# youshyee/CoSA

Measured on AMD Instinct MI355X. Metric: training images/sec at 448x448 ViT-B, higher is better.
Workload: dtype bf16; 1 GPU; VOC12 21-class, ViT-B/16 bf16, batch 16/GPU x 448x448, teacher 3 scales x 2 flips + student fwd/bwd + cam2mask x2 + 5 losses + AdamW + EMA; global_batch=16, parallelism=dp1, defer_groups=1, grid_policy=full grid

## Files before the change

### cosa_amd/csrc/gemm_kernels.hip

```cpp
#include "kernels.hpp"
#include "op16.hpp"
#include "c8.hpp"
#include "c4.hpp"
#include <cstdlib>

namespace cosa {
namespace {

typedef float f32x4 __attribute__((ext_vector_type(4)));

constexpr int BM = 128, BN = 128, BK = 64;
constexpr int TILE_BYTES = 128 * BK * 2;
constexpr int STAGE_BYTES = 2 * TILE_BYTES;
constexpr int CT_LD = 272;

enum { EPI_BIAS = 0, EPI_GELU = 1, EPI_RESIDUAL = 2 };

__device__ __forceinline__ float gelu_erf(float x)
{
    const float z = __builtin_fabsf(x) * 0.70710678118654752f;
    const float t = __builtin_amdgcn_rcpf(__builtin_fmaf(0.3275911f, z, 1.0f));
    float p = __builtin_fmaf(1.061405429f, t, -1.453152027f);
    p = __builtin_fmaf(p, t, 1.421413741f);
    p = __builtin_fmaf(p, t, -0.284496736f);
    p = __builtin_fmaf(p, t, 0.254829592f);
    p = p * t;
    const float e = __builtin_amdgcn_exp2f(-z * z * 1.4426950408889634f);
    const float erf_abs = __builtin_fmaf(-p, e, 1.0f);
    const float erfx = __builtin_copysignf(erf_abs, x);
    return 0.5f * x * (1.0f + erfx);
}

#define COSA_SPLIT_OPAQUE(a, b) asm volatile("" : "+v"(a), "+v"(b))

typedef __attribute__((address_space(3))) void lds_void;
typedef const __attribute__((address_space(1))) void gbl_void;

__device__ __forceinline__ void stage_tile(const op16 *__restrict__ src, int row0, int nrows, int ld, int k0,
                                           unsigned char *lds_tile, int wave, int lane)
{
#pragma unroll
    for (int i = 0; i < 4; i++) {
        const int q = wave * 4 + i;
        const int row = 8 * q + (lane >> 3);
        const int s = (lane & 7) ^ (row & 7);
        int grow = row0 + row;
        grow = grow < nrows ? grow : nrows - 1;
        const op16 *g = src + (size_t)grow * ld + k0 + s * 8;
        __builtin_amdgcn_global_load_lds((gbl_void *)g, (lds_void *)(lds_tile + q * 1024), 16, 0, 0);
    }
}

struct SplitGeom { int Kp; };
__device__ __forceinline__ int split_tile_x(int kt, int Kp) { return kt <= 2 * Kp ? kt : kt - 2 * Kp - 1; }
__device__ __forceinline__ int split_tile_w(int kt, int Kp) { return kt < Kp ? kt : (kt < 2 * Kp ? kt - Kp : (kt == 2 * Kp ? kt : kt - Kp - 1)); }

__device__ __forceinline__ bool c8_is_f8(int kt, int Kp) { return kt > Kp; }
__device__ __forceinline__ int c8_tile_x(int kt, int Kp) { return kt < Kp ? kt : (kt == Kp ? 2 * Kp : kt - 1); }
__device__ __forceinline__ int c8_tile_w(int kt, int Kp)
{
    const int Kh = Kp >> 1;
    return kt < Kp ? kt : (kt == Kp ? 2 * Kp : (kt <= Kp + Kh ? kt + Kh - 1 : kt - Kh - 1));
}
typedef int c8_i32x8 __attribute__((ext_vector_type(8)));
typedef int c8_i32x4 __attribute__((ext_vector_type(4)));
__device__ __forceinline__ c8_i32x8 c8_cat(op16x8 lo, op16x8 hi)
{
    return __builtin_shufflevector(__builtin_bit_cast(c8_i32x4, lo), __builtin_bit_cast(c8_i32x4, hi), 0, 1, 2, 3, 4, 5, 6, 7);
}
constexpr int kC8ScaleW = 0x7f7f7f7f;
constexpr int kC8ScaleX = 0x74747474;
#define COSA_MFMA_C8(a8, b8, c) __builtin_amdgcn_mfma_scale_f32_16x16x128_f8f6f4(a8, b8, c, 1, 1, 0, kC8ScaleW, 0, kC8ScaleX)

template <int OA, int OB>
__device__ __forceinline__ f32x4 mfma_c4(c8_i32x8 a4, c8_i32x8 b4, f32x4 c, int sa, int sb)
{
    return __builtin_amdgcn_mfma_scale_f32_16x16x128_f8f6f4(a4, b4, c, 4, 4, OA, sa, OB, sb);
}
__device__ __forceinline__ c8_i32x8 c4_op(op16x8 v)
{
    const c8_i32x4 t = __builtin_bit_cast(c8_i32x4, v);
    return (c8_i32x8){t[0], t[1], t[2], t[3], 0, 0, 0, 0};
}
__device__ __forceinline__ float c4_max4(float v)
{
    const unsigned u = __builtin_bit_cast(unsigned, v);
    const auto a = __builtin_amdgcn_permlane16_swap(u, u, false, false);
    const unsigned m = a[0] > a[1] ? a[0] : a[1];
// ... 24 lines not shown
        if (m0 >= M) return;
    } else {
        const int nwg = tiles_m * tiles_n;
        int wg = blockIdx.x;
        {
            const int q = nwg >> 3, r = nwg & 7, xcd = wg & 7, idx = wg >> 3;
            wg = (xcd < r ? xcd * (q + 1) : r * (q + 1) + (xcd - r) * q) + idx;
        }
        const int tm = wg / tiles_n, tn = wg - tm * tiles_n;
        m0 = tm * BM;
        n0 = tn * BN;
    }
    const int wr = wave >> 1, wc = wave & 1;

    f32x4 acc[4][4];
    const bool tail = tail_o0 >= 0;
#pragma unroll
    for (int i = 0; i < 4; i++)
#pragma unroll
        for (int j = 0; j < 4; j++) {
            acc[i][j] = (f32x4){0.f, 0.f, 0.f, 0.f};
            if (tail) {
                const int nl = (wave >> 1) * 64 + 16 * i + 4 * (lane >> 4), ml = (wave & 1) * 64 + 16 * j + (lane & 15);
                if (EPI == EPI_RESIDUAL) {
                    if (m0 + ml < M) acc[i][j] = *reinterpret_cast<const f32x4 *>(R + (size_t)(m0 + ml) * N + n0 + nl);
                } else {
#pragma unroll
                    for (int r = 0; r < 4; r++) acc[i][j][r] = (float)bias[n0 + nl + r];
                }
            }
        }

    const int Kp = K / BK;
    const int nk = SPLIT == 1 ? 3 * Kp + 1 : (SPLIT == 3 ? 2 * Kp + 1 : Kp);
    auto tile_x = [&](int kt) { return SPLIT == 1 ? split_tile_x(kt, Kp) : (SPLIT == 3 ? c8_tile_x(kt, Kp) : kt); };
    auto tile_w = [&](int kt) { return SPLIT == 1 ? split_tile_w(kt, Kp) : (SPLIT == 3 ? c8_tile_w(kt, Kp) : kt); };
    stage_tile(W, n0, N, ld, 0, smem, wave, lane);
    stage_tile(X, m0, M, ld, 0, smem + TILE_BYTES, wave, lane);
    asm volatile("s_waitcnt vmcnt(0)" ::: "memory");
    __syncthreads();

    const int frow = lane & 15, fq = lane >> 4;
    for (int kt = 0; kt < nk; kt++) {
        unsigned char *cur = smem + (kt & 1) * STAGE_BYTES;
        unsigned char *nxt = smem + ((kt + 1) & 1) * STAGE_BYTES;
        if (kt + 1 < nk) {
            stage_tile(W, n0, N, ld, tile_w(kt + 1) * BK, nxt, wave, lane);
            stage_tile(X, m0, M, ld, tile_x(kt + 1) * BK, nxt + TILE_BYTES, wave, lane);
        }
        const unsigned char *At = cur + (wr * 64) * 128;
        const unsigned char *Bt = cur + TILE_BYTES + (wc * 64) * 128;
        if (SPLIT == 3 && kt > Kp) {
            op16x8 a2[4][2], b2[4][2];
#pragma unroll
            for (int i = 0; i < 4; i++) {
                const int row = i * 16 + frow;
#pragma unroll
                for (int ks = 0; ks < 2; ks++) {
                    const int slot = ((fq + 4 * ks) ^ (row & 7)) << 4;
                    a2[i][ks] = *reinterpret_cast<const op16x8 *>(At + row * 128 + slot);
                    b2[i][ks] = *reinterpret_cast<const op16x8 *>(Bt + row * 128 + slot);
                }
            }
#pragma unroll
            for (int i = 0; i < 4; i++) {
                const c8_i32x8 a8 = c8_cat(a2[i][0], a2[i][1]);
#pragma unroll
                for (int j = 0; j < 4; j++) acc[i][j] = COSA_MFMA_C8(a8, c8_cat(b2[j][0], b2[j][1]), acc[i][j]);
            }
        } else
#pragma unroll
        for (int ks = 0; ks < 2; ks++) {
            op16x8 a[4], b[4];
#pragma unroll
            for (int i = 0; i < 4; i++) {
// ... 94 lines not shown
        V5_FENCE();                           \
        __builtin_amdgcn_s_barrier();         \
        V5_FENCE();                           \
    } while (0)

typedef unsigned u32x2 __attribute__((ext_vector_type(2)));
typedef unsigned u32x4 __attribute__((ext_vector_type(4)));

template <int EPI, int SPLIT = 0, int FR = 4>
__global__ __launch_bounds__(512, 1) void gemm_bf16_v6_kernel(const op16 *__restrict__ X, const op16 *__restrict__ W,
                                                             const op16 *__restrict__ bias, const float *__restrict__ R,
                                                             void *__restrict__ Yv, int M, int N, int K, int tiles_m, int tiles_n,
                                                             unsigned long long *__restrict__ stamps, int ld, int ldy, void *__restrict__ Y2v, int ntiles_run,
                                                             const unsigned char *__restrict__ xsc, const unsigned char *__restrict__ wsc, unsigned char *__restrict__ ysc)
{
    if (stamps && threadIdx.x == 0) atomicMin(&stamps[2 * (blockIdx.x & 63)], __builtin_amdgcn_s_memrealtime());
    constexpr bool RES = EPI == EPI_RESIDUAL;
    constexpr int ES = RES ? 4 : 2;
    constexpr int FL = 0x00020000;
    static_assert(FR == 4 || (FR == 3 && SPLIT == 0), "FR: 16-feature fragments per wave and W half (tile width 64 FR)");
    constexpr bool C8 = SPLIT == 3;
    constexpr bool C8OUT = C8 && EPI == EPI_GELU;
    constexpr bool C4 = SPLIT == 4;
    constexpr bool C4OUT = C4 && EPI == EPI_GELU;
    constexpr bool CX = C8 || C4;
    static_assert(!C4 || FR == 4, "fp16c4: 256-wide jobs only (the scale tensors are laid out for them)");
    constexpr int TN = 64 * FR, HN = 32 * FR, WN = 16 * FR;
    extern __shared__ __attribute__((aligned(16))) unsigned char smem[];
    const int tid = threadIdx.x, wave = tid >> 6, lane = tid & 63;
    const int wr = wave >> 2, wc = wave & 3;
    const int frow = lane & 15, fq = lane >> 4;
    const int Kp = K / BK;
    const int Kq = Kp >> 1;
    const int nk = SPLIT == 1 ? 3 * Kp + 1 : (C8 ? 2 * Kp + 1 : (C4 ? Kp + 1 + Kq : Kp));
    const int ntiles = tiles_m * tiles_n, G = gridDim.x;
    const int cq = ntiles >> 3, cr = ntiles & 7;
    unsigned char *Yb = static_cast<unsigned char *>(Yv);

    auto tile_of = [&](int o, int &m0_, int &n0_) {
        const int xcd = o & 7, idx = o >> 3;
        const int t = (xcd < cr ? xcd * (cq + 1) : cr * (cq + 1) + (xcd - cr) * cq) + idx;
        const int tm = t / tiles_n;
        m0_ = tm * 256;
        n0_ = (t - tm * tiles_n) * TN;
    };
    auto descX = [&](int m0_) {
        int rows = M - m0_;
        rows = rows > 256 ? 256 : rows;
        return __builtin_amdgcn_make_buffer_rsrc((void *)(X + (size_t)m0_ * ld), 0, rows * ld * 2, FL);
    };
    auto descW = [&](int n0_) { return __builtin_amdgcn_make_buffer_rsrc((void *)(W + (size_t)n0_ * ld), 0, TN * ld * 2, FL); };
    auto descY2 = [&](int m0_, int n0_) {
        int rows = M - m0_;
        rows = rows > 256 ? 256 : rows;
        return __builtin_amdgcn_make_buffer_rsrc((void *)(static_cast<unsigned char *>(Y2v) + ((size_t)m0_ * ldy + n0_) * 2), 0, (rows * ldy - n0_) * 2, FL);
    };
    auto descY = [&](int m0_, int n0_) {
        int rows = M - m0_;
        rows = rows > 256 ? 256 : rows;
        return __builtin_amdgcn_make_buffer_rsrc((void *)(Yb + ((size_t)m0_ * ldy + n0_) * ES), 0, (rows * ldy - n0_) * ES, FL);
    };
    auto descR = [&](int m0_, int n0_) {
        int rows = M - m0_;
        rows = rows > 256 ? 256 : rows;
        const unsigned long long p = (unsigned long long)(R + (size_t)m0_ * N + n0_);
        return (u32x4){(unsigned)p, (unsigned)(p >> 32) & 0xffffu, (unsigned)((rows * N - n0_) * 4), (unsigned)FL};
    };
// ... 3 lines not shown
    __amdgpu_buffer_rsrc_t sXr = dead, sWr = dead, sYr = dead;
    if (C4) {
        sXr = __builtin_amdgcn_make_buffer_rsrc((void *)xsc, 0, tiles_m * Kq * 2048, FL);
        sWr = __builtin_amdgcn_make_buffer_rsrc((void *)wsc, 0, tiles_n * Kq * 2048, FL);
        if (C4OUT) sYr = __builtin_amdgcn_make_buffer_rsrc((void *)ysc, 0, tiles_m * (N >> 7) * 2048, FL);
    }
    const unsigned sc_rd_x = (unsigned)(((wc * 16 + frow) * 4 + fq) * 8), sc_rd_w = (unsigned)(4096 + ((wr * 16 + frow) * 4 + fq) * 16);
    const unsigned sc_wr_y = (unsigned)((((wc * 16 + frow) * 4 + (fq & 1) + 2 * (fq >> 1)) * 8) + wr);
    u32x2 sxv = {0, 0};
    u32x4 swv = {0, 0, 0, 0};
#define V6_SCDMA(c)                                                                                                    \
    do {                                                                                                               \
        const int c_ = (c);                                                                                            \
        const __amdgpu_buffer_rsrc_t rs_ = wave_u < 4 ? sXr : sWr;                                                     \
        const int so_ = wave_u < 4 ? (((m0 >> 8) * Kq + 2 * c_) * 2048 + wave_u * 1024) : (((n0 >> 8) * Kq + 2 * c_) * 2048 + (wave_u - 4) * 1024); \
        __builtin_amdgcn_raw_ptr_buffer_load_lds(rs_, (lds_void *)(smem + kLdsBytesV5 + (c_ & 1) * 8192 + wave_u * 1024), 16, lane * 16, so_, 0, 0); \
    } while (0)
#define V6_LDSC(q)                                                                                                     \
    do {                                                                                                               \
        const unsigned char *sb_ = smem + kLdsBytesV5 + (((q) >> 1) & 1) * 8192 + ((q) & 1) * 2048;                    \
        sxv = *reinterpret_cast<const u32x2 *>(sb_ + sc_rd_x);                                                         \
        swv = *reinterpret_cast<const u32x4 *>(sb_ + sc_rd_w);            \
    } while (0)

    unsigned vo[2][2], voW[2][2];
    {
        const int sw = ((lane & 7) ^ (lane >> 3)) * 8;
#pragma unroll
        for (int h = 0; h < 2; h++)
#pragma unroll
            for (int i = 0; i < 2; i++) {
                const int rl = 8 * (2 * wave + i) + (lane >> 3);
                vo[h][i] = (unsigned)(((h * 128 + rl) * ld + sw) * 2);
                voW[h][i] = FR == 4 ? vo[h][i] : (rl < HN ? (unsigned)(((h * HN + rl) * ld + sw) * 2) : 0x7ffff000u);
            }
    }
    const unsigned voY0 = RES ? (unsigned)(((wc * 32 + frow) * ldy + wr * WN + 4 * fq) * 4)
                              : (unsigned)(((wc * 32 + frow) * ldy + wr * WN + (fq & 1) * 16 + 4 * (fq & 2)) * 2);
    const unsigned voY3 = (unsigned)((32 + 4 * fq - (fq & 1) * 16 - 4 * (fq & 2)) * 2);
    const unsigned fo16m = (unsigned)((wr * WN + 16 * (fq & 1) + 32 * (fq >> 1)) - 2 * (wr * WN + (fq & 1) * 16 + 4 * (fq & 2)));

    constexpr bool STG = FR == 4 && EPI != EPI_GELU;
    constexpr int STGW = C4 ? 2048 : 4096;
    const unsigned stg0 = (unsigned)(kLdsBytesV5 + (C4 ? kC4ScaleLds : 0) + wave * STGW);
    const unsigned stg_w = stg0 + frow * 128 + ((((RES ? fq : (fq & 1) * 2 + (fq >> 1))) ^ (frow & 7)) << 4);
    const unsigned stg_r = stg0 + (lane >> 3) * 128 + (((lane & 7) ^ ((lane >> 3) & 7)) << 4);
    const unsigned voS = (unsigned)(((wc * 32 + (lane >> 3)) * ldy + wr * WN) * ES + (lane & 7) * 16);
#define V6_STG_WR(u4, e, plane) *reinterpret_cast<u32x4 *>(smem + ((stg_w ^ ((e) * 64)) + (plane) * 2048)) = (u4)
#define V6_STG_RD(it, plane) (*reinterpret_cast<const u32x4 *>(smem + (stg_r + (it) * 1024 + (plane) * 2048)))
    const int ldy_es = __builtin_amdgcn_readfirstlane(ldy * ES);
#define V6_VOY(g4)                                                                                                   \
    ({                                                                                                               \
        unsigned r_ = voY0;                                                                                          \
        if ((g4) != 0)                                                                                               \
            asm volatile("v_add_u32 %0, %1, %2" : "=v"(r_) : "s"((((g4) >> 1) * 128 + ((g4) & 1) * 16) * ldy_es), "v"(voY0));  \
        r_;                                                                                                          \
    })
#define V6_STG_OFF(qb, jj, it)                                                                                       \
    ({                                                                                                               \
        unsigned r_ = voS;                                                                                           \
        if ((qb) * 128 + (jj) * 16 + (it) * 8 != 0)                                                                  \
            asm volatile("v_add_u32 %0, %1, %2" : "=v"(r_) : "s"(((qb) * 128 + (jj) * 16 + (it) * 8) * ldy_es), "v"(voS));  \
        r_;                                                                                                          \
    })

    int o = blockIdx.x;
    int m0, n0, m1 = 0, n1 = 0, pn0 = 0, pm0 = 0;
    tile_of(o, m0, n0);
    bool has_next = o + G < ntiles_run;
    if (has_next) tile_of(o + G, m1, n1);
    __amdgpu_buffer_rsrc_t cX = descX(m0), cW = descW(n0), cY = descY(m0, n0), pY = cY;
    __amdgpu_buffer_rsrc_t cY2 = SPLIT == 2 ? descY2(m0, n0) : cY, pY2 = cY2;
    __amdgpu_buffer_rsrc_t nX = has_next ? descX(m1) : dead, nW = has_next ? descW(n1) : dead;
    u32x4 cR = {0, 0, 0, 0}, nR = {0, 0, 0, 0};
    if (RES) {
        cR = descR(m0, n0);
        if (has_next) nR = descR(m1, n1);
    }
    bool have_prev = false;

    u32x2 bb[2][4];
    const unsigned bias_lane = (unsigned)((wr * WN + 4 * fq) * 2);
#define V6_LOAD_BIAS(nbase)                                                                               \
    if (!CX) _Pragma("unroll") for (int a_ = 0; a_ < 2; a_++) _Pragma("unroll") for (int i_ = 0; i_ < FR; i_++) {  \
        const op16 *p_ = bias + (nbase) + a_ * HN + i_ * 16;                                              \
        asm volatile("global_load_dwordx2 %0, %1, %2" : "=v"(bb[a_][i_]) : "v"(bias_lane), "s"(p_) : "memory"); \
    }

#define V6_STAGE(which, kt, bsel)                                                                                      \
    do {                                                                                                               \
        const int kt_ = (kt);                                                                                          \
        const bool own_ = kt_ < nk;                                                                                    \
        const __amdgpu_buffer_rsrc_t rs_ = ((which) & 1) ? (own_ ? cW : nW) : (own_ ? cX : nX);                        \
        const int t_ = own_ ? kt_ : kt_ - nk;                                                                          \
        const int so_ = (SPLIT == 1 ? (((which) & 1) ? split_tile_w(t_, Kp) : split_tile_x(t_, Kp))                       \
                         : (C8 ? (((which) & 1) ? c8_tile_w(t_, Kp) : c8_tile_x(t_, Kp)) : (C4 ? c8_tile_x(t_, Kp) : t_))) * 128;   \
        unsigned char *dst_ = smem + (bsel) * V5_BUF + (which) * V5_HALF + (2 * wave) * 1024;                          \
        __builtin_amdgcn_raw_ptr_buffer_load_lds(rs_, (lds_void *)dst_, 16, ((which) & 1) ? voW[(which) >> 1][0] : vo[(which) >> 1][0], so_, 0, 0);           \
        __builtin_amdgcn_raw_ptr_buffer_load_lds(rs_, (lds_void *)(dst_ + 1024), 16, ((which) & 1) ? voW[(which) >> 1][1] : vo[(which) >> 1][1], so_, 0, 0);  \
    } while (0)

    f32x4 acc[8][4];
#define V6_RLOAD(qa, qb, rsR)                                                                                        \
    _Pragma("unroll") for (int ii = 0; ii < FR; ii++) _Pragma("unroll") for (int jj = 0; jj < 2; jj++)               \
        asm volatile("buffer_load_dwordx4 %0, %1, %2, %3 offen" : "=v"(acc[(qa) * 4 + ii][(qb) * 2 + jj])           \
                     : "v"(V6_VOY((qb) * 2 + jj)), "s"(rsR), "s"(((qa) * HN + ii * 16) * 4) : "memory");

    V6_LOAD_BIAS(n0);
    if (RES) {
        V6_RLOAD(0, 0, cR);
        V6_RLOAD(0, 1, cR);
        V6_RLOAD(1, 1, cR);
        V6_RLOAD(1, 0, cR);
    }
    V5_FENCE();
    V6_STAGE(0, 0, 0);
    V6_STAGE(1, 0, 0);
    V6_STAGE(2, 0, 0);
    V6_STAGE(3, 0, 0);
    V6_STAGE(0, 1, 1);
    V6_STAGE(1, 1, 1);
    V6_STAGE(2, 1, 1);
    asm volatile("s_waitcnt vmcnt(6)" ::: "memory");
    V5_BARRIER();
    if (wr == 1) V5_BARRIER();

    const int lo0 = frow * 128 + ((fq ^ (frow & 7)) << 4), lo1 = lo0 ^ 64;
    const unsigned char *rdW0 = smem + V5_HALF + wr * (WN * 128) + lo0, *rdW1 = smem + V5_HALF + wr * (WN * 128) + lo1;
    const unsigned char *rdX0 = smem + wc * 4096 + lo0, *rdX1 = smem + wc * 4096 + lo1;
    op16x8 a[4][2], x0[2][2], x1[2][2];

#define V6_LDW(q, buf)                                                                     \
    _Pragma("unroll") for (int blk = 0; blk < FR; blk++) {                                 \
        const int o_ = (buf) * V5_BUF + (q) * 2 * V5_HALF + blk * 2048;                    \
        a[blk][0] = *reinterpret_cast<const op16x8 *>(rdW0 + o_);                          \
        a[blk][1] = *reinterpret_cast<const op16x8 *>(rdW1 + o_);                          \
    }
#define V6_LDX(dst, q, buf)                                                                \
    _Pragma("unroll") for (int blk = 0; blk < 2; blk++) {                                  \
        const int o_ = (buf) * V5_BUF + (q) * 2 * V5_HALF + blk * 2048;                    \
        dst[blk][0] = *reinterpret_cast<const op16x8 *>(rdX0 + o_);                        \
        dst[blk][1] = *reinterpret_cast<const op16x8 *>(rdX1 + o_);                        \
    }
#define V6_EPI(qa, qb, rsY)                                                                                         \
    if (RES && STG) {          \
        _Pragma("unroll") for (int jj = 0; jj < 2; jj++) _Pragma("unroll") for (int p2 = 0; p2 < 2; p2++) {         \
            _Pragma("unroll") for (int e_ = 0; e_ < 2; e_++) {                                                      \
                const int ii = 2 * p2 + e_;                                                                         \
                const unsigned lo_ = CX ? 0u : bb[qa][ii][0], hi_ = CX ? 0u : bb[qa][ii][1];                        \
                const f32x4 bv_ = CX ? (f32x4){0.f, 0.f, 0.f, 0.f} : (f32x4){op16_lo(lo_), op16_hi(lo_), op16_lo(hi_), op16_hi(hi_)};  \
                const f32x4 o4_ = acc[(qa) * 4 + ii][(qb) * 2 + jj] + bv_;                                          \
                V6_STG_WR(__builtin_bit_cast(u32x4, o4_), e_, 0);                                                   \
            }                                                                                                       \
            _Pragma("unroll") for (int it_ = 0; it_ < 2; it_++)                                                     \
                __builtin_amdgcn_raw_buffer_store_b128(V6_STG_RD(it_, 0), rsY, V6_STG_OFF(qb, jj, it_) + ((qa) * HN + p2 * 32) * 4, 0, 0); \
        }                                                                                                           \
    } else if (RES) {                                                                                               \
        _Pragma("unroll") for (int ii = 0; ii < FR; ii++) {                                                         \
            const unsigned lo_ = CX ? 0u : bb[qa][ii][0], hi_ = CX ? 0u : bb[qa][ii][1];                            \
            const f32x4 bv_ = CX ? (f32x4){0.f, 0.f, 0.f, 0.f} : (f32x4){op16_lo(lo_), op16_hi(lo_), op16_lo(hi_), op16_hi(hi_)};  \
            _Pragma("unroll") for (int jj = 0; jj < 2; jj++) {                                                      \
                const f32x4 o4_ = acc[(qa) * 4 + ii][(qb) * 2 + jj] + bv_;                                          \
                __builtin_amdgcn_raw_buffer_store_b128(__builtin_bit_cast(u32x4, o4_), rsY,                         \
                                                       V6_VOY((qb) * 2 + jj) + ((qa) * HN + ii * 16) * 4, 0, 0);     \
            }                                                                                                       \
        }                                                                                                           \
    } else {                                                                                                        \
    unsigned c8l_[2][2], c8h_[2][2];        \
    unsigned c4d_[2][2]; int c4e_[2][2];   \
    _Pragma("unroll") for (int jj = 0; jj < 2; jj++) _Pragma("unroll") for (int pr = 0; pr < 2; pr++) {             \
        if (FR == 3 && pr == 1) {                                                  \
            f32x4 v2_ = acc[(qa) * 4 + 2][(qb) * 2 + jj];                                                           \
            if (EPI == EPI_GELU) { _Pragma("unroll") for (int r = 0; r < 4; r++) v2_[r] = gelu_erf(v2_[r]); }       \
// ... 88 lines not shown
                const unsigned g0_ = x0_[0], g1_ = x1_[0], g2_ = x0_[1], g3_ = x1_[1];       \
                const u32x4 blk_ = {(g0_ & 0xffffu) | (g1_ << 16), (g2_ & 0xffffu) | (g3_ << 16),                    \
                                    (g0_ >> 16) | (g1_ & 0xffff0000u), (g2_ >> 16) | (g3_ & 0xffff0000u)};          \
                const int jn0_ = (&rsY == &pY) ? pn0 : n0, jm0_ = (&rsY == &pY) ? pm0 : m0;                         \
                __builtin_amdgcn_raw_buffer_store_b128(blk_, rsY, V6_VOY((qb) * 2 + jj) + fo16m, 2 * N - jn0_ + (qa) * HN, 0); \
                const int el_ = fq == 0 ? c4e_[0][0] : (fq == 1 ? c4e_[0][1] : (fq == 2 ? c4e_[1][0] : c4e_[1][1])); \
                __builtin_amdgcn_raw_buffer_store_b8((unsigned char)c4_scale_byte(el_, 0), sYr, sc_wr_y + ((qb) * 2 + jj) * 2, \
                                                     (((jm0_ >> 8) * (N >> 7) + (jn0_ >> 7) + (qa)) << 11), 0);   \
            }                                                                                                       \
        }                                                                                                           \
        if (STG && pr == 1) {        \
            _Pragma("unroll") for (int it_ = 0; it_ < 2; it_++) {                                                   \
                const unsigned vo_ = V6_STG_OFF(qb, jj, it_) + (qa) * HN * 2;                                 \
                if (SPLIT == 2) {                   \
                    __builtin_amdgcn_raw_buffer_store_b128(V6_STG_RD(it_, 1), rsY, vo_, 0, 0);                      \
                    __builtin_amdgcn_raw_buffer_store_b128(V6_STG_RD(it_, 0), (&rsY == &pY) ? pY2 : cY2, vo_, 0, 0); \
                } else {                                                                                            \
                    __builtin_amdgcn_raw_buffer_store_b128(V6_STG_RD(it_, 0), rsY, vo_, 0, 0);                      \
                    if (SPLIT == 1) __builtin_amdgcn_raw_buffer_store_b128(V6_STG_RD(it_, 1), rsY, vo_ + N * 2, 0, 0); \
                }                                                                                                   \
            }                                                                                                       \
        }                                                                                                           \
    }                                                                                                               \
    }
#define V6_C4ROW(qa, xf, qb, i, ks)                                                                                 \
    do {                                                                                                            \
        const c8_i32x8 a4_ = c4_op(a[i][ks]);                                                                       \
        const int sa_ = (int)swv[(qa) * 2 + ((i) >> 1)], sb_ = (int)sxv[qb];                                        \
        acc[(qa) * 4 + (i)][(qb) * 2] = mfma_c4<((i) & 1) * 2 + (ks), (ks)>(a4_, c4_op(xf[0][ks]), acc[(qa) * 4 + (i)][(qb) * 2], sa_, sb_);             \
        acc[(qa) * 4 + (i)][(qb) * 2 + 1] = mfma_c4<((i) & 1) * 2 + (ks), 2 + (ks)>(a4_, c4_op(xf[1][ks]), acc[(qa) * 4 + (i)][(qb) * 2 + 1], sa_, sb_); \
    } while (0)
#define V6_MMA(qa, xf, qb, FIRST, F8)                                                                               \
    do {                                                                                                            \
        if ((F8) == 2) {       \
            V6_C4ROW(qa, xf, qb, 0, 0); V6_C4ROW(qa, xf, qb, 1, 0); V6_C4ROW(qa, xf, qb, 2, 0); V6_C4ROW(qa, xf, qb, 3, 0);  \
            V6_C4ROW(qa, xf, qb, 0, 1); V6_C4ROW(qa, xf, qb, 1, 1); V6_C4ROW(qa, xf, qb, 2, 1); V6_C4ROW(qa, xf, qb, 3, 1);  \
        } else if (F8) {       \
            _Pragma("unroll") for (int i = 0; i < FR; i++) {                                                        \
                const c8_i32x8 a8_ = c8_cat(a[i][0], a[i][1]);                                                      \
                _Pragma("unroll") for (int j = 0; j < 2; j++)                                                       \
                    acc[(qa) * 4 + i][(qb) * 2 + j] = COSA_MFMA_C8(a8_, c8_cat(xf[j][0], xf[j][1]), acc[(qa) * 4 + i][(qb) * 2 + j]); \
            }                                                                                                       \
        } else                                                                                                      \
        _Pragma("unroll") for (int ks = 0; ks < 2; ks++)                                                            \
            _Pragma("unroll") for (int i = 0; i < FR; i++) {                                                        \
                f32x4 cb_;                                                                                          \
                if ((FIRST) && ks == 0 && !RES) {                                                                   \
                    const unsigned lo_ = CX ? 0u : bb[qa][i][0], hi_ = CX ? 0u : bb[qa][i][1];       \
                    cb_[0] = op16_lo(lo_);                                                                          \
                    cb_[1] = op16_hi(lo_);                                                                          \
                    cb_[2] = op16_lo(hi_);                                                                          \
                    cb_[3] = op16_hi(hi_);                                                                          \
                }                                                                                                   \
                _Pragma("unroll") for (int j = 0; j < 2; j++)                                                       \
                    acc[(qa) * 4 + i][(qb) * 2 + j] = COSA_MFMA_16x16x32(                      \
                        a[i][ks], xf[j][ks], ((FIRST) && ks == 0 && !RES) ? cb_ : acc[(qa) * 4 + i][(qb) * 2 + j], 0, 0, 0); \
            }                                                                                                       \
    } while (0)
#define V6_MSECTION_BEGIN()                                    \
    V5_BARRIER();                                              \
    asm volatile("s_waitcnt lgkmcnt(0)" ::: "memory");         \
    __builtin_amdgcn_s_setprio(1)
#define V6_MSECTION_END()                                      \
    __builtin_amdgcn_s_setprio(0);                             \
    V5_BARRIER()

#define V6_WAIT(n) asm volatile("s_waitcnt vmcnt(" #n ")" ::: "memory")
#define V6_TILE(t, FIRST, LAST, F8)                                                                                 \
    do {                                                                                                            \
        const int b_ = g & 1;                                                                                       \
                                                                                             \
        if ((F8) == 2) { V6_LDSC((t) - Kp - 1); V5_FENCE(); }                                                       \
        V6_LDX(x0, 0, b_);                                                                                          \
        V5_FENCE();                                                                                                 \
        V6_LDW(0, b_);                                                                                              \
        if (!RES && (LAST) && has_next) { V6_LOAD_BIAS(n1); }                                                       \
        V5_FENCE();                                                                                                 \
        if (C4 && !(FIRST) && !(LAST)) {      \
            const int d_ = (t) - (Kp - 1);                                                                          \
            if (d_ >= 0 && !(d_ & 1) && (d_ >> 1) < (Kq >> 1)) V6_SCDMA(d_ >> 1);                                   \
            V5_FENCE();                                                                                             \
        }                                                                                                           \
        V6_STAGE(3, (t) + 1, b_ ^ 1);                                                                               \
        V5_FENCE();                                                                                                 \
        asm volatile("s_waitcnt lgkmcnt(8)" ::: "memory");                                                          \
        V6_MSECTION_BEGIN();                                                                                        \
        if (RES && (FIRST)) { if (FR == 4) V6_WAIT(38); else V6_WAIT(30); V5_FENCE(); }                             \
        if ((FIRST) && have_prev) {                                                                                 \
            V6_EPI(1, 0, pY);                                                                                       \
            if (RES) { V5_FENCE(); V6_RLOAD(1, 0, cR); V6_LOAD_BIAS(n0); V5_FENCE(); }                              \
        }                                                                                                           \
        V6_MMA(0, x0, 0, FIRST, F8);                                                                                    \
        V6_MSECTION_END();                                                                                          \
                                                                                             \
        V6_LDX(x1, 1, b_);                                                                                          \
        V6_STAGE(0, (t) + 2, b_);                                                                                   \
        V6_MSECTION_BEGIN();                                                                                        \
        if (RES && (FIRST)) { if (FR == 4) V6_WAIT(46); else V6_WAIT(36); V5_FENCE(); }                             \
        if (LAST) {                                                                                                 \
            V6_EPI(0, 0, cY);                                                                                       \
            if (RES && has_next) { V5_FENCE(); V6_RLOAD(0, 0, nR); V5_FENCE(); }                                    \
        }                                                                                                           \
        V6_MMA(0, x1, 1, FIRST, F8);                                                                                    \
        V6_MSECTION_END();                                                                                          \
                                                                                             \
        V6_LDW(1, b_);                                                                                              \
        V6_STAGE(1, (t) + 2, b_);                                                                                   \
        V6_MSECTION_BEGIN();                                                                                        \
        if (RES && (FIRST)) { if (FR == 4) V6_WAIT(30); else V6_WAIT(24); V5_FENCE(); }                             \
        if (LAST) {                                                                                                 \
            V6_EPI(0, 1, cY);                                                                                       \
            if (RES && has_next) { V5_FENCE(); V6_RLOAD(0, 1, nR); V5_FENCE(); }                                    \
        }                                                                                                           \
        V6_MMA(1, x1, 1, FIRST, F8);                                                                                    \
        V6_MSECTION_END();                                                                                          \
                                                                                             \
        V6_STAGE(2, (t) + 2, b_);                                                                                   \
        V5_FENCE();                                                                                                 \
        if ((LAST) && RES) { if (FR == 4) V6_WAIT(38); else V6_WAIT(30); }                                          \
        else if ((LAST) && (C8OUT || C4OUT)) V6_WAIT(22);       \
        else if (LAST) V6_WAIT(14);                                                                                 \
        else V6_WAIT(6);                                                                                            \
        V6_MSECTION_BEGIN();                                                                                        \
        if (LAST) {                                                                                                 \
            V6_EPI(1, 1, cY);                                                                                       \
            if (RES && has_next) { V5_FENCE(); V6_RLOAD(1, 1, nR); V5_FENCE(); }                                    \
        }                                                                                                           \
        V6_MMA(1, x0, 0, FIRST, F8);                                                                                    \
        V6_MSECTION_END();                                                                                          \
        g++;                                                                                                        \
    } while (0)

    int g = 0;
    while (true) {
        if (C8) {
            V6_TILE(0, 1, 0, 0);
            for (int t = 1; t <= Kp; t++) V6_TILE(t, 0, 0, 0);
            for (int t = Kp + 1; t < nk - 1; t++) V6_TILE(t, 0, 0, 1);
            V6_TILE(nk - 1, 0, 1, 1);
        } else if (C4) {
            V6_TILE(0, 1, 0, 0);
            for (int t = 1; t <= Kp; t++) V6_TILE(t, 0, 0, 0);
            for (int t = Kp + 1; t < nk - 1; t++) V6_TILE(t, 0, 0, 2);
            V6_TILE(nk - 1, 0, 1, 2);
        } else {
            V6_TILE(0, 1, 0, 0);
            for (int t = 1; t < nk - 1; t++) V6_TILE(t, 0, 0, 0);
            V6_TILE(nk - 1, 0, 1, 0);
        }
        if (!has_next) break;
        pn0 = n0;
        pm0 = m0;
        pY = cY;
        pY2 = cY2;
        have_prev = true;
        o += G;
        m0 = m1;
        n0 = n1;
        cX = nX;
        cW = nW;
        cY = descY(m0, n0);
        if (SPLIT == 2) cY2 = descY2(m0, n0);
        cR = nR;
        has_next = o + G < ntiles_run;
        if (has_next) {
            tile_of(o + G, m1, n1);
            nX = descX(m1);
            nW = descW(n1);
            if (RES) nR = descR(m1, n1);
        } else {
            nX = dead;
            nW = dead;
        }
    }
    V6_EPI(1, 0, cY);
    if (wr == 0) V5_BARRIER();
    asm volatile("s_waitcnt vmcnt(0)" ::: "memory");
// ... 451 lines not shown
                for (int j = 0; j < 4; j++)
                    acc[i][j] = COSA_MFMA_16x16x32(a[i], b[j], acc[i][j], 0, 0, 0);
        }
        asm volatile("s_waitcnt vmcnt(0)" ::: "memory");
        __syncthreads();
    }
    unsigned char *Ct = smem;
#pragma unroll
    for (int i = 0; i < 4; i++) {
        const int nl = wr * 64 + 16 * i + 4 * fq;
#pragma unroll
        for (int j = 0; j < 4; j++) {
            const int ml = wc * 64 + 16 * j + frow;
            op16x4 v;
#pragma unroll
            for (int r = 0; r < 4; r++) {
                float t = acc[i][j][r];
                if (relu) t = t > 0.f ? t : 0.f;
                v[r] = (op16)t;
            }
            *reinterpret_cast<op16x4 *>(Ct + ml * CT_LD + nl * 2) = v;
        }
    }
    __syncthreads();
#pragma unroll
    for (int c = tid; c < BM * 16; c += 256) {
        const int ml = c >> 4, s2 = c & 15;
        if (m0 + ml < M)
            *reinterpret_cast<uint4 *>(Y + (size_t)(m0 + ml) * Cout + n0 + s2 * 8) = *reinterpret_cast<const uint4 *>(Ct + ml * CT_LD + s2 * 16);
    }
}

constexpr size_t kLdsBytes = 128 * (BN * 4 + 16) > 2 * STAGE_BYTES ? 128 * (BN * 4 + 16) : 2 * STAGE_BYTES;

template <int D>
__global__ __launch_bounds__(256) void layernorm_kernel(const float *__restrict__ x, const op16 *__restrict__ g,
                                                       const op16 *__restrict__ b, op16 *__restrict__ y, float *__restrict__ y32,
                                                       int rows, float eps)
{
    const int row = blockIdx.x * 4 + (threadIdx.x >> 6);
    if (row >= rows) return;
    const int lane = threadIdx.x & 63;
    constexpr int PER = D / 64 / 4;
    const float4 *xr = reinterpret_cast<const float4 *>(x + (size_t)row * D);
    float4 v[PER];
    float s = 0.f;
#pragma unroll
    for (int i = 0; i < PER; i++) { v[i] = xr[lane + 64 * i]; s += v[i].x + v[i].y + v[i].z + v[i].w; }
#pragma unroll
    for (int o = 32; o > 0; o >>= 1) s += __shfl_xor(s, o, 64);
    const float mean = s * (1.0f / D);
    float q = 0.f;
#pragma unroll
    for (int i = 0; i < PER; i++) {
        const float a = v[i].x - mean, c = v[i].y - mean, d = v[i].z - mean, e = v[i].w - mean;
        q += a * a + c * c + d * d + e * e;
    }
#pragma unroll
    for (int o = 32; o > 0; o >>= 1) q += __shfl_xor(q, o, 64);
    const float rstd = rsqrtf(q * (1.0f / D) + eps);
#pragma unroll
    for (int i = 0; i < PER; i++) {
        const int c0 = (lane + 64 * i) * 4;
        const op16x4 gg = *reinterpret_cast<const op16x4 *>(g + c0);
        const op16x4 bb = *reinterpret_cast<const op16x4 *>(b + c0);
        float o0 = (v[i].x - mean) * rstd * (float)gg[0] + (float)bb[0];
// ... 38 lines not shown
template <int EPI, int SPLIT = 0, int FR = 4>
static int launch_v6(const op16 *x, const op16 *w, const op16 *b, const float *residual, void *Y, int M, int N, int K, hipStream_t st,
                     int ld = 0, int ldy = 0, void *Y2 = nullptr, const unsigned char *xsc = nullptr, const unsigned char *wsc = nullptr,
                     unsigned char *ysc = nullptr)
{
    constexpr size_t lds_bytes = kLdsBytesV5 + (SPLIT == 4 ? kC4ScaleLds + kStageLdsC4 : kStageLds);
    static bool attr_done = false;
    if (!attr_done) {
        COSA_HIP_CHECK(hipFuncSetAttribute((const void *)gemm_bf16_v6_kernel<EPI, SPLIT, FR>, hipFuncAttributeMaxDynamicSharedMemorySize, (int)lds_bytes));
        attr_done = true;
    }
    const int tiles_m = (M + 255) / 256, tiles_n = N / (64 * FR);
    const int ntiles = tiles_m * tiles_n;
    const int grid = ntiles < 256 ? ntiles : 256;
    constexpr int tail_max = 48;
    int run = ntiles;
    const int rem = ntiles % 256, rounds_up = (ntiles + 255) / 256;
    constexpr bool can_tail = FR == 4 && (SPLIT == 0 || SPLIT == 1 || (SPLIT == 3 && EPI == EPI_RESIDUAL));
    if (can_tail && ntiles > 256 && rem != 0 && rem <= tail_max && (256 - rem) * 10 > 256 * rounds_up)
        run = ntiles - rem;
    const bool balanced = g_gemm_balanced_grid != 0;
    int grid_b = grid;
    if (balanced && run > 256 && M < 40000) {
        const int rounds = (run + 255) / 256;
        grid_b = ((run + rounds - 1) / rounds + 7) / 8 * 8;
        grid_b = grid_b > 256 ? 256 : grid_b;
    }
    hipLaunchKernelGGL((gemm_bf16_v6_kernel<EPI, SPLIT, FR>), dim3(grid_b), dim3(512), lds_bytes, st, x, w, b, residual, Y, M, N, K, tiles_m, tiles_n,
                       g_gemm_stamp_slot, ld ? ld : K, ldy ? ldy : N, Y2, run, xsc, wsc, ysc);
    g_gemm_stamp_slot = nullptr;
    COSA_LAUNCH_CHECK();
    if constexpr (can_tail) {
        if (run < ntiles) {
            constexpr int tail_lds = (SPLIT == 1 && 2 * BM * CT_LD > (int)kLdsBytes) ? 2 * BM * CT_LD : (int)kLdsBytes;
            static bool tail_attr = false;
            if (!tail_attr) {
                COSA_HIP_CHECK(hipFuncSetAttribute((const void *)gemm_bf16_kernel<EPI, SPLIT>, hipFuncAttributeMaxDynamicSharedMemorySize, tail_lds));
                tail_attr = true;
            }
            hipLaunchKernelGGL((gemm_bf16_kernel<EPI, SPLIT>), dim3(4 * (ntiles - run)), dim3(256), tail_lds, st, x, w, b, residual, Y, M, N, K, tiles_m, tiles_n,
                               ld ? ld : K, ldy ? ldy : N, static_cast<void *>(nullptr), run);
            COSA_LAUNCH_CHECK();
        }
    }
    return COSA_OK;
}

extern "C" int cosa_gemm_bf16(const void *X, const void *W, const void *bias, const float *residual, void *Y,
                              int M, int N, int K, int epilogue, void *stream)
{
    struct ClearSlot { ~ClearSlot() { g_gemm_stamp_slot = nullptr; } } clear_slot_;
    COSA_REQUIRE(X && W && bias && Y, "cosa_gemm_bf16: null pointer");
    COSA_REQUIRE(M > 0 && N > 0 && K > 0, "cosa_gemm_bf16: bad shape");
    COSA_REQUIRE(N % BN == 0 && K % BK == 0, "cosa_gemm_bf16: N must be a multiple of 128 and K of 64 (got N=%d K=%d)", N, K);
    COSA_REQUIRE(epilogue >= 0 && epilogue <= 2, "cosa_gemm_bf16: unknown epilogue");
    COSA_REQUIRE(epilogue != EPI_RESIDUAL || residual, "cosa_gemm_bf16: residual epilogue needs the residual pointer");
    const int tiles_m = (M + BM - 1) / BM, tiles_n = N / BN;
    const dim3 grid(tiles_m * tiles_n), blk(256);
    hipStream_t st = as_stream(stream);
    const op16 *x = static_cast<const op16 *>(X), *w = static_cast<const op16 *>(W), *b = static_cast<const op16 *>(bias);
    const bool fits_v5 = N % 256 == 0 && M >= 256 && (size_t)(M + 256) * K * 2 < 0x7fffffffull && (size_t)N * K * 2 < 0x7fffffffull;
    constexpr int big_m = 4096;
    const bool fits_v6 = fits_v5 && K >= 128 && (epilogue != EPI_RESIDUAL || g_gemm_variant == 6 || g_gemm_variant == 9 || g_gemm_variant == 0);
    if (fits_v6 && N % 192 == 0 && (g_gemm_variant == 9 || (g_gemm_variant == 0 && M >= big_m))) {
        constexpr int wide_max = 48;
        const long tm = (M + 255) / 256, n4 = tm * (N / 256), n3 = tm * (N / 192);
        const double r4 = (n4 > 256 && n4 % 256 != 0 && n4 % 256 <= wide_max) ? (double)(n4 / 256) + 0.1 : (double)((n4 + 255) / 256);
// ... 18 lines not shown
    }
    switch (epilogue) {
    case EPI_BIAS:
        hipLaunchKernelGGL(gemm_bf16_kernel<EPI_BIAS>, grid, blk, kLdsBytes, st, x, w, b, residual, Y, M, N, K, tiles_m, tiles_n, K, N, nullptr);
        break;
    case EPI_GELU:
        hipLaunchKernelGGL(gemm_bf16_kernel<EPI_GELU>, grid, blk, kLdsBytes, st, x, w, b, residual, Y, M, N, K, tiles_m, tiles_n, K, N, nullptr);
        break;
    default:
        hipLaunchKernelGGL(gemm_bf16_kernel<EPI_RESIDUAL>, grid, blk, kLdsBytes, st, x, w, b, residual, Y, M, N, K, tiles_m, tiles_n, K, N, nullptr);
        break;
    }
    COSA_LAUNCH_CHECK();
    return COSA_OK;
}

extern "C" int cosa_gemm_bf16x3(const void *Xs, const void *Ws, const void *zeros, const float *residual, void *Y,
                                int M, int N, int K, int epilogue, int ldy, void *stream)
{
    struct ClearSlot { ~ClearSlot() { g_gemm_stamp_slot = nullptr; } } clear_slot_;
    COSA_REQUIRE(Xs && Ws && zeros && Y, "cosa_gemm_bf16x3: null pointer");
    COSA_REQUIRE(M > 0 && N > 0 && K > 0 && N % BN == 0 && K % BK == 0, "cosa_gemm_bf16x3: N %% 128 and K %% 64 must be 0 (got N=%d K=%d)", N, K);
    COSA_REQUIRE(epilogue >= 0 && epilogue <= 2, "cosa_gemm_bf16x3: unknown epilogue");
    COSA_REQUIRE(epilogue != EPI_RESIDUAL || residual, "cosa_gemm_bf16x3: residual epilogue needs the residual pointer");
    COSA_REQUIRE(epilogue == EPI_RESIDUAL ? ldy == N : (ldy >= 2 * N && ldy % 8 == 0), "cosa_gemm_bf16x3: ldy must be N (fp32 out) or >= 2N (split out)");
    const int ld = 2 * K + 64;
    hipStream_t st = as_stream(stream);
    const op16 *x = static_cast<const op16 *>(Xs), *w = static_cast<const op16 *>(Ws), *b = static_cast<const op16 *>(zeros);
    if (N % 256 == 0 && M >= 4096 && (size_t)(M + 256) * ld * 2 < 0x7fffffffull * 8 && (size_t)N * ld * 2 < 0x7fffffffull) {
        if (epilogue == EPI_BIAS) return launch_v6<EPI_BIAS, 1>(x, w, b, residual, Y, M, N, K, st, ld, ldy);
        if (epilogue == EPI_GELU) return launch_v6<EPI_GELU, 1>(x, w, b, residual, Y, M, N, K, st, ld, ldy);
        return launch_v6<EPI_RESIDUAL, 1>(x, w, b, residual, Y, M, N, K, st, ld, ldy);
    }
    constexpr int kLdsSplit = 2 * BM * CT_LD > (int)kLdsBytes ? 2 * BM * CT_LD : (int)kLdsBytes;
    static bool attr_done = false;
    if (!attr_done) {
        COSA_HIP_CHECK(hipFuncSetAttribute((const void *)gemm_bf16_kernel<EPI_BIAS, 1>, hipFuncAttributeMaxDynamicSharedMemorySize, kLdsSplit));
        COSA_HIP_CHECK(hipFuncSetAttribute((const void *)gemm_bf16_kernel<EPI_GELU, 1>, hipFuncAttributeMaxDynamicSharedMemorySize, kLdsSplit));
        COSA_HIP_CHECK(hipFuncSetAttribute((const void *)gemm_bf16_kernel<EPI_RESIDUAL, 1>, hipFuncAttributeMaxDynamicSharedMemorySize, kLdsSplit));
        attr_done = true;
    }
    const int tiles_m = (M + BM - 1) / BM, tiles_n = N / BN;
    const dim3 grid(tiles_m * tiles_n), blk(256);
    switch (epilogue) {
    case EPI_BIAS:
        hipLaunchKernelGGL((gemm_bf16_kernel<EPI_BIAS, 1>), grid, blk, kLdsSplit, st, x, w, b, residual, Y, M, N, K, tiles_m, tiles_n, ld, ldy, nullptr);
        break;
    case EPI_GELU:
        hipLaunchKernelGGL((gemm_bf16_kernel<EPI_GELU, 1>), grid, blk, kLdsSplit, st, x, w, b, residual, Y, M, N, K, tiles_m, tiles_n, ld, ldy, nullptr);
        break;
    default:
        hipLaunchKernelGGL((gemm_bf16_kernel<EPI_RESIDUAL, 1>), grid, blk, kLdsSplit, st, x, w, b, residual, Y, M, N, K, tiles_m, tiles_n, ld, ldy, nullptr);
        break;
    }
    COSA_LAUNCH_CHECK();
    return COSA_OK;
}

#if COSA_OP_F16
extern "C" int cosa_gemm_f16c8(const void *Xs, const void *Ws, const void *zeros, const float *residual, void *Y,
                               int M, int N, int K, int epilogue, int ldy, void *stream)
{
    struct ClearSlot { ~ClearSlot() { g_gemm_stamp_slot = nullptr; } } clear_slot_;
    COSA_REQUIRE(Xs && Ws && zeros && Y, "cosa_gemm_f16c8: null pointer");
    COSA_REQUIRE(M > 0 && N > 0 && K > 0 && N % 256 == 0 && K % 128 == 0, "cosa_gemm_f16c8: N %% 256 == 0 and K %% 128 == 0 required (got M=%d N=%d K=%d)", M, N, K);
    COSA_REQUIRE(epilogue >= 0 && epilogue <= 2, "cosa_gemm_f16c8: unknown epilogue");
    COSA_REQUIRE(epilogue != EPI_RESIDUAL || residual, "cosa_gemm_f16c8: residual epilogue needs the residual pointer");
// ... 210 lines not shown
```

Baseline: 209.2 images/s.

## Fuse split-bf16x3 GEMM hi/lo passes into single K sweep reusing staged tiles

Restructures the 3-term split-precision (bf16x3) GEMM path. Before, it ran three sequential K passes over hi/lo tiles (3*Kp+1 steps). Now each K step stages the hi and lo halves of X and W together and issues hi*hi, hi*lo and lo*hi MFMAs from the same LDS data, which cuts redundant reloads of the hi operands. This changes the LDS layout (64-byte rows, a new swizzle), the stage ordering and the wait counts in the v6 pipelined kernel. It also doubles the stage footprint for the fallback kernel, which could lower occupancy.

Result: faster. 221.7 images/s (median of 6 runs) (+6.0%).

```diff
diff --git a/cosa_amd/csrc/gemm_kernels.hip b/cosa_amd/csrc/gemm_kernels.hip
--- a/cosa_amd/csrc/gemm_kernels.hip
+++ b/cosa_amd/csrc/gemm_kernels.hip
@@ -51,9 +51,7 @@
     }
 }
 
-struct SplitGeom { int Kp; };
-__device__ __forceinline__ int split_tile_x(int kt, int Kp) { return kt <= 2 * Kp ? kt : kt - 2 * Kp - 1; }
-__device__ __forceinline__ int split_tile_w(int kt, int Kp) { return kt < Kp ? kt : (kt < 2 * Kp ? kt - Kp : (kt == 2 * Kp ? kt : kt - Kp - 1)); }
+__device__ __forceinline__ int x3_step_col(int t, int lo, int K) { return t == 0 ? 2 * K : lo * K + (t - 1) * 32; }
 
 __device__ __forceinline__ bool c8_is_f8(int kt, int Kp) { return kt > Kp; }
 __device__ __forceinline__ int c8_tile_x(int kt, int Kp) { return kt < Kp ? kt : (kt == Kp ? 2 * Kp : kt - 1); }
@@ -144,15 +142,71 @@
         }
 
     const int Kp = K / BK;
-    const int nk = SPLIT == 1 ? 3 * Kp + 1 : (SPLIT == 3 ? 2 * Kp + 1 : Kp);
-    auto tile_x = [&](int kt) { return SPLIT == 1 ? split_tile_x(kt, Kp) : (SPLIT == 3 ? c8_tile_x(kt, Kp) : kt); };
-    auto tile_w = [&](int kt) { return SPLIT == 1 ? split_tile_w(kt, Kp) : (SPLIT == 3 ? c8_tile_w(kt, Kp) : kt); };
-    stage_tile(W, n0, N, ld, 0, smem, wave, lane);
-    stage_tile(X, m0, M, ld, 0, smem + TILE_BYTES, wave, lane);
-    asm volatile("s_waitcnt vmcnt(0)" ::: "memory");
-    __syncthreads();
+    [[maybe_unused]] const int nk = SPLIT == 3 ? 2 * Kp + 1 : Kp;
+    [[maybe_unused]] auto tile_x = [&](int kt) { return SPLIT == 3 ? c8_tile_x(kt, Kp) : kt; };
+    [[maybe_unused]] auto tile_w = [&](int kt) { return SPLIT == 3 ? c8_tile_w(kt, Kp) : kt; };
+    if constexpr (SPLIT == 1) {
+        const int frow = lane & 15, fq = lane >> 4;
+        constexpr int STAGE3 = 4 * TILE_BYTES;
+        auto stage3 = [&](int st, unsigned char *buf) {
+            const int c_hi = st == 0 ? 2 * K : (st - 1) * BK;
+            stage_tile(W, n0, N, ld, c_hi, buf, wave, lane);
+            stage_tile(X, m0, M, ld, c_hi, buf + TILE_BYTES, wave, lane);
+            if (st != 0) {
+                stage_tile(W, n0, N, ld, K + c_hi, buf + 2 * TILE_BYTES, wave, lane);
+                stage_tile(X, m0, M, ld, K + c_hi, buf + 3 * TILE_BYTES, wave, lane);
+            }
+        };
+        stage3(0, smem);
+        asm volatile("s_waitcnt vmcnt(0)" ::: "memory");
+        __syncthreads();
+        for (int st = 0; st <= Kp; st++) {
+            unsigned char *cur = smem + (st & 1) * STAGE3;
+            if (st < Kp) stage3(st + 1, smem + ((st + 1) & 1) * STAGE3);
+            const unsigned char *At = cur + (wr * 64) * 128;
+            const unsigned char *Bt = cur + TILE_BYTES + (wc * 64) * 128;
+#pragma unroll
+            for (int ks = 0; ks < 2; ks++) {
+                if (st == 0 && ks == 1) break;
+                op16x8 ah[4], bh[4], al[4], bl[4];
+#pragma unroll
+                for (int i = 0; i < 4; i++) {
+                    const int row = i * 16 + frow;
+                    const int slot = ((fq + 4 * ks) ^ (row & 7)) << 4;
+                    ah[i] = *reinterpret_cast<const op16x8 *>(At + row * 128 + slot);
+                    bh[i] = *reinterpret_cast<const op16x8 *>(Bt + row * 128 + slot);
+                    if (st != 0) {
+                        al[i] = *reinterpret_cast<const op16x8 *>(At + 2 * TILE_BYTES + row * 128 + slot);
+                        bl[i] = *reinterpret_cast<const op16x8 *>(Bt + 2 * TILE_BYTES + row * 128 + slot);
+                    }
+                }
+#pragma unroll
+                for (int i = 0; i < 4; i++)
+#pragma unroll
+                    for (int j = 0; j < 4; j++) acc[i][j] = COSA_MFMA_16x16x32(ah[i], bh[j], acc[i][j], 0, 0, 0);
+                if (st != 0) {
+#pragma unroll
+                    for (int i = 0; i < 4; i++)
+#pragma unroll
+                        for (int j = 0; j < 4; j++) acc[i][j] = COSA_MFMA_16x16x32(ah[i], bl[j], acc[i][j], 0, 0, 0);
+#pragma unroll
+                    for (int i = 0; i < 4; i++)
+#pragma unroll
+                        for (int j = 0; j < 4; j++) acc[i][j] = COSA_MFMA_16x16x32(al[i], bh[j], acc[i][j], 0, 0, 0);
+                }
+            }
+            asm volatile("s_waitcnt vmcnt(0)" ::: "memory");
+            __syncthreads();
+        }
+    } else {
+        stage_tile(W, n0, N, ld, 0, smem, wave, lane);
+        stage_tile(X, m0, M, ld, 0, smem + TILE_BYTES, wave, lane);
+        asm volatile("s_waitcnt vmcnt(0)" ::: "memory");
+        __syncthreads();
+    }
 
     const int frow = lane & 15, fq = lane >> 4;
+    if constexpr (SPLIT != 1)
     for (int kt = 0; kt < nk; kt++) {
         unsigned char *cur = smem + (kt & 1) * STAGE_BYTES;
         unsigned char *nxt = smem + ((kt + 1) & 1) * STAGE_BYTES;
@@ -313,7 +367,8 @@
     const int frow = lane & 15, fq = lane >> 4;
     const int Kp = K / BK;
     const int Kq = Kp >> 1;
-    const int nk = SPLIT == 1 ? 3 * Kp + 1 : (C8 ? 2 * Kp + 1 : (C4 ? Kp + 1 + Kq : Kp));
+    constexpr bool X3 = SPLIT == 1;
+    const int nk = X3 ? 2 * Kp + 1 : (C8 ? 2 * Kp + 1 : (C4 ? Kp + 1 + Kq : Kp));
     const int ntiles = tiles_m * tiles_n, G = gridDim.x;
     const int cq = ntiles >> 3, cr = ntiles & 7;
     unsigned char *Yb = static_cast<unsigned char *>(Yv);
@@ -383,6 +438,10 @@
             for (int i = 0; i < 2; i++) {
                 const int rl = 8 * (2 * wave + i) + (lane >> 3);
                 vo[h][i] = (unsigned)(((h * 128 + rl) * ld + sw) * 2);
+                if (X3) {
+                    const int r3 = 16 * (2 * wave + i) + (lane >> 2);
+                    vo[h][i] = (unsigned)((r3 * ld + ((lane & 3) ^ ((r3 >> 2) & 3)) * 8) * 2);
+                }
                 voW[h][i] = FR == 4 ? vo[h][i] : (rl < HN ? (unsigned)(((h * HN + rl) * ld + sw) * 2) : 0x7ffff000u);
             }
     }
@@ -442,10 +501,11 @@
     do {                                                                                                               \
         const int kt_ = (kt);                                                                                          \
         const bool own_ = kt_ < nk;                                                                                    \
-        const __amdgpu_buffer_rsrc_t rs_ = ((which) & 1) ? (own_ ? cW : nW) : (own_ ? cX : nX);                        \
+        __amdgpu_buffer_rsrc_t rs_ = ((which) & 1) ? (own_ ? cW : nW) : (own_ ? cX : nX);                              \
         const int t_ = own_ ? kt_ : kt_ - nk;                                                                          \
-        const int so_ = (SPLIT == 1 ? (((which) & 1) ? split_tile_w(t_, Kp) : split_tile_x(t_, Kp))                       \
-                         : (C8 ? (((which) & 1) ? c8_tile_w(t_, Kp) : c8_tile_x(t_, Kp)) : (C4 ? c8_tile_x(t_, Kp) : t_))) * 128;   \
+        const int so_ = X3 ? x3_step_col(t_, (which) >> 1, K) * 2                                                      \
+                           : (C8 ? (((which) & 1) ? c8_tile_w(t_, Kp) : c8_tile_x(t_, Kp)) : (C4 ? c8_tile_x(t_, Kp) : t_)) * 128;   \
+        if (X3 && (which) >= 2 && t_ == 0) rs_ = dead;        \
         unsigned char *dst_ = smem + (bsel) * V5_BUF + (which) * V5_HALF + (2 * wave) * 1024;                          \
         __builtin_amdgcn_raw_ptr_buffer_load_lds(rs_, (lds_void *)dst_, 16, ((which) & 1) ? voW[(which) >> 1][0] : vo[(which) >> 1][0], so_, 0, 0);           \
         __builtin_amdgcn_raw_ptr_buffer_load_lds(rs_, (lds_void *)(dst_ + 1024), 16, ((which) & 1) ? voW[(which) >> 1][1] : vo[(which) >> 1][1], so_, 0, 0);  \
@@ -469,27 +529,34 @@
     V6_STAGE(1, 0, 0);
     V6_STAGE(2, 0, 0);
     V6_STAGE(3, 0, 0);
-    V6_STAGE(0, 1, 1);
-    V6_STAGE(1, 1, 1);
-    V6_STAGE(2, 1, 1);
-    asm volatile("s_waitcnt vmcnt(6)" ::: "memory");
+    if (X3) {
+        V6_STAGE(0, 1, 1);
+        V6_STAGE(2, 1, 1);
+        asm volatile("s_waitcnt vmcnt(4)" ::: "memory");
+    } else {
+        V6_STAGE(0, 1, 1);
+        V6_STAGE(1, 1, 1);
+        V6_STAGE(2, 1, 1);
+        asm volatile("s_waitcnt vmcnt(6)" ::: "memory");
+    }
     V5_BARRIER();
     if (wr == 1) V5_BARRIER();
 
-    const int lo0 = frow * 128 + ((fq ^ (frow & 7)) << 4), lo1 = lo0 ^ 64;
-    const unsigned char *rdW0 = smem + V5_HALF + wr * (WN * 128) + lo0, *rdW1 = smem + V5_HALF + wr * (WN * 128) + lo1;
-    const unsigned char *rdX0 = smem + wc * 4096 + lo0, *rdX1 = smem + wc * 4096 + lo1;
+    const int lo0 = X3 ? frow * 64 + ((fq ^ (frow >> 2)) << 4) : frow * 128 + ((fq ^ (frow & 7)) << 4), lo1 = X3 ? lo0 + 2 * V5_HALF : lo0 ^ 64;
+    constexpr int RB = X3 ? 64 : 128;
+    const unsigned char *rdW0 = smem + V5_HALF + wr * (WN * RB) + lo0, *rdW1 = smem + V5_HALF + wr * (WN * RB) + lo1;
+    const unsigned char *rdX0 = smem + wc * (32 * RB) + lo0, *rdX1 = smem + wc * (32 * RB) + lo1;
     op16x8 a[4][2], x0[2][2], x1[2][2];
 
 #define V6_LDW(q, buf)                                                                     \
     _Pragma("unroll") for (int blk = 0; blk < FR; blk++) {                                 \
-        const int o_ = (buf) * V5_BUF + (q) * 2 * V5_HALF + blk * 2048;                    \
+        const int o_ = (buf) * V5_BUF + (q) * (X3 ? 128 * RB : 2 * V5_HALF) + blk * 16 * RB; \
         a[blk][0] = *reinterpret_cast<const op16x8 *>(rdW0 + o_);                          \
         a[blk][1] = *reinterpret_cast<const op16x8 *>(rdW1 + o_);                          \
     }
 #define V6_LDX(dst, q, buf)                                                                \
     _Pragma("unroll") for (int blk = 0; blk < 2; blk++) {                                  \
-        const int o_ = (buf) * V5_BUF + (q) * 2 * V5_HALF + blk * 2048;                    \
+        const int o_ = (buf) * V5_BUF + (q) * (X3 ? 128 * RB : 2 * V5_HALF) + blk * 16 * RB; \
         dst[blk][0] = *reinterpret_cast<const op16x8 *>(rdX0 + o_);                        \
         dst[blk][1] = *reinterpret_cast<const op16x8 *>(rdX1 + o_);                        \
     }
@@ -644,7 +711,22 @@
     } while (0)
 #define V6_MMA(qa, xf, qb, FIRST, F8)                                                                               \
     do {                                                                                                            \
-        if ((F8) == 2) {       \
+        if (X3) {              \
+            _Pragma("unroll") for (int p_ = 0; p_ < ((F8) ? 1 : 3); p_++)                                               \
+                _Pragma("unroll") for (int i = 0; i < 4; i++) {                                                         \
+                    f32x4 cb_;                                                                                          \
+                    if ((FIRST) && p_ == 0 && !RES) {                                                                   \
+                        const unsigned lo_ = bb[qa][i][0], hi_ = bb[qa][i][1];                                          \
+                        cb_[0] = op16_lo(lo_);                                                                          \
+                        cb_[1] = op16_hi(lo_);                                                                          \
+                        cb_[2] = op16_lo(hi_);                                                                          \
+                        cb_[3] = op16_hi(hi_);                                                                          \
+                    }                                                                                                   \
+                    _Pragma("unroll") for (int j = 0; j < 2; j++)                                                       \
+                        acc[(qa) * 4 + i][(qb) * 2 + j] = COSA_MFMA_16x16x32(                                           \
+                            a[i][p_ == 2], xf[j][p_ == 1], ((FIRST) && p_ == 0 && !RES) ? cb_ : acc[(qa) * 4 + i][(qb) * 2 + j], 0, 0, 0); \
+                }                                                                                                       \
+        } else if ((F8) == 2) {       \
             V6_C4ROW(qa, xf, qb, 0, 0); V6_C4ROW(qa, xf, qb, 1, 0); V6_C4ROW(qa, xf, qb, 2, 0); V6_C4ROW(qa, xf, qb, 3, 0);  \
             V6_C4ROW(qa, xf, qb, 0, 1); V6_C4ROW(qa, xf, qb, 1, 1); V6_C4ROW(qa, xf, qb, 2, 1); V6_C4ROW(qa, xf, qb, 3, 1);  \
         } else if (F8) {       \
@@ -693,7 +775,7 @@
             if (d_ >= 0 && !(d_ & 1) && (d_ >> 1) < (Kq >> 1)) V6_SCDMA(d_ >> 1);                                   \
             V5_FENCE();                                                                                             \
         }                                                                                                           \
-        V6_STAGE(3, (t) + 1, b_ ^ 1);                                                                               \
+        if (X3) V6_STAGE(1, (t) + 1, b_ ^ 1); else V6_STAGE(3, (t) + 1, b_ ^ 1);                                    \
         V5_FENCE();                                                                                                 \
         asm volatile("s_waitcnt lgkmcnt(8)" ::: "memory");                                                          \
         V6_MSECTION_BEGIN();                                                                                        \
@@ -706,7 +788,7 @@
         V6_MSECTION_END();                                                                                          \
                                                                                              \
         V6_LDX(x1, 1, b_);                                                                                          \
-        V6_STAGE(0, (t) + 2, b_);                                                                                   \
+        if (X3) V6_STAGE(3, (t) + 1, b_ ^ 1); else V6_STAGE(0, (t) + 2, b_);                                        \
         V6_MSECTION_BEGIN();                                                                                        \
         if (RES && (FIRST)) { if (FR == 4) V6_WAIT(46); else V6_WAIT(36); V5_FENCE(); }                             \
         if (LAST) {                                                                                                 \
@@ -717,7 +799,7 @@
         V6_MSECTION_END();                                                                                          \
                                                                                              \
         V6_LDW(1, b_);                                                                                              \
-        V6_STAGE(1, (t) + 2, b_);                                                                                   \
+        if (X3) V6_STAGE(0, (t) + 2, b_); else V6_STAGE(1, (t) + 2, b_);                                            \
         V6_MSECTION_BEGIN();                                                                                        \
         if (RES && (FIRST)) { if (FR == 4) V6_WAIT(30); else V6_WAIT(24); V5_FENCE(); }                             \
         if (LAST) {                                                                                                 \
@@ -729,7 +811,8 @@
                                                                                              \
         V6_STAGE(2, (t) + 2, b_);                                                                                   \
         V5_FENCE();                                                                                                 \
-        if ((LAST) && RES) { if (FR == 4) V6_WAIT(38); else V6_WAIT(30); }                                          \
+        if (X3) { if ((LAST) && RES) V6_WAIT(36); else if (LAST) V6_WAIT(20); else V6_WAIT(4); }                    \
+        else if ((LAST) && RES) { if (FR == 4) V6_WAIT(38); else V6_WAIT(30); }                                     \
         else if ((LAST) && (C8OUT || C4OUT)) V6_WAIT(22);       \
         else if (LAST) V6_WAIT(14);                                                                                 \
         else V6_WAIT(6);                                                                                            \
@@ -755,6 +838,10 @@
             for (int t = 1; t <= Kp; t++) V6_TILE(t, 0, 0, 0);
             for (int t = Kp + 1; t < nk - 1; t++) V6_TILE(t, 0, 0, 2);
             V6_TILE(nk - 1, 0, 1, 2);
+        } else if (X3) {
+            V6_TILE(0, 1, 0, 1);
+            for (int t = 1; t < nk - 1; t++) V6_TILE(t, 0, 0, 0);
+            V6_TILE(nk - 1, 0, 1, 0);
         } else {
             V6_TILE(0, 1, 0, 0);
             for (int t = 1; t < nk - 1; t++) V6_TILE(t, 0, 0, 0);
@@ -1272,6 +1359,7 @@
 }
 
 constexpr size_t kLdsBytes = 128 * (BN * 4 + 16) > 2 * STAGE_BYTES ? 128 * (BN * 4 + 16) : 2 * STAGE_BYTES;
+constexpr int kLdsSplit3 = 2 * 4 * TILE_BYTES;
 
 template <int D>
 __global__ __launch_bounds__(256) void layernorm_kernel(const float *__restrict__ x, const op16 *__restrict__ g,
@@ -1376,7 +1464,7 @@
     COSA_LAUNCH_CHECK();
     if constexpr (can_tail) {
         if (run < ntiles) {
-            constexpr int tail_lds = (SPLIT == 1 && 2 * BM * CT_LD > (int)kLdsBytes) ? 2 * BM * CT_LD : (int)kLdsBytes;
+            constexpr int tail_lds = SPLIT == 1 ? kLdsSplit3 : (int)kLdsBytes;
             static bool tail_attr = false;
             if (!tail_attr) {
                 COSA_HIP_CHECK(hipFuncSetAttribute((const void *)gemm_bf16_kernel<EPI, SPLIT>, hipFuncAttributeMaxDynamicSharedMemorySize, tail_lds));
@@ -1461,7 +1549,7 @@
         if (epilogue == EPI_GELU) return launch_v6<EPI_GELU, 1>(x, w, b, residual, Y, M, N, K, st, ld, ldy);
         return launch_v6<EPI_RESIDUAL, 1>(x, w, b, residual, Y, M, N, K, st, ld, ldy);
     }
-    constexpr int kLdsSplit = 2 * BM * CT_LD > (int)kLdsBytes ? 2 * BM * CT_LD : (int)kLdsBytes;
+    constexpr int kLdsSplit = kLdsSplit3;
     static bool attr_done = false;
     if (!attr_done) {
         COSA_HIP_CHECK(hipFuncSetAttribute((const void *)gemm_bf16_kernel<EPI_BIAS, 1>, hipFuncAttributeMaxDynamicSharedMemorySize, kLdsSplit));
```
